# raulmur/ORB_SLAM

Measured on AMD Instinct MI355X. Metric: frames/s ORB extract+match @640x480, 1000 kp, higher is better.
Workload: dtype u8; 1 GPU; vga: 640x480 grayscale stream, 8 levels, nFeatures 1000, S-blocks frames, extract + Hamming top-2 match vs previous frame (BASELINE.json configs[1] + the frame-to-frame match of the metric); resident_frames_per_gpu=2048, lanes=4, parity_checked_frames=0, parity_mismatches=0, library_build_id=255c35022344858e, lane_placement=2

## Files before the change

orb_slam_amd/csrc/k_describe_od.hip:

```cpp
#include <algorithm>
#include <type_traits>

#include "orbx_device.h"

namespace orbx {

constexpr int OD_KPW = 4;
constexpr int OD_PITCH = 48, OD_ROWS = 43;
constexpr int OD_WIN_BYTES = OD_PITCH * OD_ROWS;
constexpr int OD_CHUNKS = OD_ROWS * 3;
constexpr int OD_WAVES = DESC_WAVES;
constexpr int OD_TAIL = 512;

typedef int v4i __attribute__((ext_vector_type(4)));
typedef float f2v __attribute__((ext_vector_type(2)));
__device__ __forceinline__ int float_bits(float v) { return __builtin_bit_cast(int, v); }
typedef const void __attribute__((address_space(1))) * gptr_t;
typedef void __attribute__((address_space(3))) * lptr_t;

constexpr int od_tap(int t) { return t >= 0 && t <= 6 ? (int)((0x12223137312212ull >> (8 * t)) & 255ull) : 0; }
constexpr uint32_t od_taps4(int t0) { return (uint32_t)od_tap(t0) | (uint32_t)od_tap(t0 + 1) << 8 | (uint32_t)od_tap(t0 + 2) << 16 | (uint32_t)od_tap(t0 + 3) << 24; }
struct OdTables {
    uint32_t mask[256];
    float pat[256][4];
    uint32_t trow[3][64][4];
    uint32_t tcol[4][64][4];
};
constexpr uint32_t c_pattern_host[256] = {
#include "orb_pattern_packed.inc"
};
constexpr OdTables make_od_tables() {
    OdTables T{};
    for (int t = 0; t < 256; t++) {
        const int r = t >> 3, c = t & 7;
        const int v = r - HALF_PATCH, av = v < 0 ? -v : v;
        const int um = r < 31 ? (int)((UMAX_NIBBLES >> (4 * (av & 15))) & 15ull) : -1;
        uint32_t mask = 0;
        for (int kk = 0; kk < 4; kk++) {
            const int u = 4 * c + kk - HALF_PATCH;
            if ((u < 0 ? -u : u) <= um) mask |= 0xFFu << (8 * kk);
        }
        T.mask[t] = mask;
        const uint32_t pk = c_pattern_host[t];
        for (int e = 0; e < 4; e++) T.pat[t][e] = (float)(int)(int8_t)(uint8_t)(pk >> (8 * e));
    }
    for (int c = 0; c < 3; c++)
        for (int l = 0; l < 64; l++)
            for (int v = 0; v < 4; v++) {
                const int n = l & 15, g = l >> 4;
                if (c < 2) T.trow[c][l][v] = od_taps4(16 * g + 4 * v - (16 * c + n) - 1);
                else T.trow[c][l][v] = g == 2 && n < 8 ? od_taps4(4 * v - n - 1) : g == 3 && n >= 8 ? od_taps4(4 * v - (n - 8) - 1) : 0u;
            }
    for (int c = 0; c < 4; c++)
        for (int l = 0; l < 64; l++)
            for (int v = 0; v < 4; v++) {
                const int n = l & 15, g = l >> 4;
                uint32_t word = 0;
                for (int h = 0; h < 2; h++) {
                    const int row = 4 * g + 2 * (v >> 1) + h;
                    const int t = c == 0 ? row - n : c == 1 ? 16 + row - n : c == 2 ? (n < 5 ? row - n : -1) : (n >= 8 && n < 13 ? row - (n - 8) : -1);
                    word |= f16_bits_scaled(blur_tap(t), (v & 1) ? 8 : 16) << (16 * h);
                }
                T.tcol[c][l][v] = word;
            }
    return T;
}
static __device__ __constant__ OdTables c_od = make_od_tables();

typedef _Float16 h8v __attribute__((ext_vector_type(8)));
typedef _Float16 h2v __attribute__((ext_vector_type(2)));
typedef float f4v __attribute__((ext_vector_type(4)));
constexpr bool OD_CVT_RNE = true;
constexpr int OD_GEN = 0, OD_EVEN = 1, OD_UP = 2;

struct OdWin { int xs, yq; uint32_t tw; bool gen; };
__device__ __forceinline__ void od_blur_windows(uint8_t* win0, int lane, int nlive, OdWin w0, OdWin w1, OdWin w2, OdWin w3, int Lw, int Lh, int Lwvec, const v4i (&Trow)[3], const v4i (&Tcol)[2], const v4i* tprow) {
    const int n16 = lane & 15, g4 = lane >> 4;
    const unsigned a_off = (unsigned)(n16 * OD_PITCH + 16 * g4);
    const unsigned a_offp = g4 == 3 ? (unsigned)(OD_WIN_BYTES + n16 * OD_PITCH + 32) : a_off;
    const unsigned o_own = (unsigned)((n16 + 3) * OD_PITCH + 4 + 4 * g4);
    const unsigned o_prow = (unsigned)((n16 >= 8 ? OD_WIN_BYTES : 0) + ((n16 & 7) + 35) * OD_PITCH + 4 + 4 * g4);
    const unsigned o_pcol = (unsigned)((g4 >= 2 ? OD_WIN_BYTES : 0) + (n16 + 3) * OD_PITCH + 36 + 4 * (g4 & 1));
    const unsigned o_corner = (unsigned)((n16 < 8 ? 2 : 0) * OD_WIN_BYTES + (g4 >= 2 ? OD_WIN_BYTES : 0) + ((n16 & 7) + 35) * OD_PITCH + 36 + 4 * (g4 & 1));
    const v4i cmid = {blurf_mid_start(), blurf_mid_start(), blurf_mid_start(), blurf_mid_start()};
    const h2v unbias = {(_Float16)-blurf_lo_bias(), (_Float16)-blurf_lo_bias()};
    auto row_pass = [&](const v4i (&A)[3], const v4i& T, v4i (&M)[3]) {
        v4i z[3];
#pragma unroll
        for (int t = 0; t < 3; t++) z[t] = __builtin_amdgcn_mfma_i32_16x16x64_i8(A[t], T, cmid, 0, 0, 0);
#pragma unroll
        for (int t = 0; t < 3; t++)
#pragma unroll
            for (int h = 0; h < 2; h++) {
                const uint32_t z0 = (uint32_t)z[t][2 * h], z1 = (uint32_t)z[t][2 * h + 1];
                M[t][2 * h] = (int)__builtin_amdgcn_perm(z1, z0, 0x06040200u);
                M[t][2 * h + 1] = __builtin_bit_cast(int, __builtin_bit_cast(h2v, __builtin_amdgcn_perm(z1, z0, 0x06050201u)) + unbias);
            }
    };
    auto epilogue = [&](auto MODE, const v4i& Ma, const v4i& Mb, const v4i& Ta, const v4i& Tb, uint8_t* dst, int xs_l, int yq_l, int cb, int ro) {
        constexpr bool gen = decltype(MODE)::value == OD_GEN, twu = decltype(MODE)::value == OD_EVEN;
        constexpr float st = (gen || twu) ? blurf_start() : blurf_start() + 0.5f;
        f4v acc = {st, st, st, st};
        acc = __builtin_amdgcn_mfma_f32_16x16x32_f16(__builtin_bit_cast(h8v, Ma), __builtin_bit_cast(h8v, Ta), acc, 0, 0, 0);
        acc = __builtin_amdgcn_mfma_f32_16x16x32_f16(__builtin_bit_cast(h8v, Mb), __builtin_bit_cast(h8v, Tb), acc, 0, 0, 0);
        float v[4] = {acc[0], acc[1], acc[2], acc[3]};
        uint32_t keep = 0;
        if (gen) {
            const int X0 = xs_l + 4 + cb;
            const bool te = X0 < Lwvec;
            uint32_t keepc = 0;
#pragma unroll
            for (int bb = 0; bb < 4; bb++) keepc |= ((unsigned)(X0 + bb) < (unsigned)Lw ? 0u : 0xFFu) << (8 * bb);
            keep = (unsigned)(yq_l - 18 + ro) < (unsigned)Lh ? keepc : 0xFFFFFFFFu;
#pragma unroll
            for (int i = 0; i < 4; i++) v[i] = te ? __builtin_rintf(v[i]) : __builtin_floorf(v[i] + 0.5f);
        } else if (!twu) {
#pragma unroll
            for (int i = 0; i < 4; i++) v[i] = __builtin_floorf(v[i]);
        } else if (!OD_CVT_RNE) {
#pragma unroll
            for (int i = 0; i < 4; i++) v[i] = __builtin_rintf(v[i]);
        }
        uint32_t o = 0;
#pragma unroll
        for (int i = 0; i < 4; i++) o = __builtin_amdgcn_cvt_pk_u8_f32(v[i], (uint32_t)i, o);
        uint32_t* d = reinterpret_cast<uint32_t*>(dst);
        if (gen) o = (o & ~keep) | (*d & keep);
        *d = o;
    };
    v4i mc[2] = {{0, 0, 0, 0}, {0, 0, 0, 0}};
    auto blur_pair = [&](auto GEN, int p, int xs0, int yq0, int xs1, int yq1) {
        uint8_t* W = win0 + 2 * p * OD_WIN_BYTES;
        v4i A0[3], A1[3];
        {
            const unsigned r0 = (unsigned)(uintptr_t)(lptr_t)(W + a_offp), r1 = (unsigned)(uintptr_t)(lptr_t)(W + OD_WIN_BYTES + a_off);
            asm volatile("ds_read_b128 %0, %6\n\tds_read_b128 %1, %6 offset:768\n\tds_read_b128 %2, %6 offset:1536\n\t"
                         "ds_read_b128 %3, %7\n\tds_read_b128 %4, %7 offset:768\n\tds_read_b128 %5, %7 offset:1536\n\ts_waitcnt lgkmcnt(0)"
                         : "=&v"(A0[0]), "=&v"(A0[1]), "=&v"(A0[2]), "=&v"(A1[0]), "=&v"(A1[1]), "=&v"(A1[2]) : "v"(r0), "v"(r1) : "memory");
        }
#pragma unroll
        for (int t = 0; t < 3; t++)
#pragma unroll
            for (int e = 0; e < 4; e++) { A0[t][e] = (int)((uint32_t)A0[t][e] ^ 0x80808080u); A1[t][e] = (int)((uint32_t)A1[t][e] ^ 0x80808080u); }
        const int xs_r = n16 >= 8 ? xs1 : xs0, yq_r = n16 >= 8 ? yq1 : yq0;
        const int xs_c = g4 >= 2 ? xs1 : xs0, yq_c = g4 >= 2 ? yq1 : yq0;
        {
            v4i MP[3];
            row_pass(A0, Trow[2], MP);
#pragma unroll
            for (int rt = 0; rt < 2; rt++)
                epilogue(GEN, MP[rt], MP[rt + 1], Tcol[0], Tcol[1], W + o_pcol + 16 * rt * OD_PITCH, xs_c, yq_c, 32 + 4 * (g4 & 1), 16 * rt + n16);
            if (p == 0) { mc[0] = MP[2]; mc[1] = MP[2]; }
            else mc[1] = MP[2];
        }
#pragma unroll
        for (int ct = 0; ct < 2; ct++) {
            v4i M0[3], M1[3];
            row_pass(A0, Trow[ct], M0);
#pragma unroll
            for (int rt = 0; rt < 2; rt++)
                epilogue(GEN, M0[rt], M0[rt + 1], Tcol[0], Tcol[1], W + o_own + (16 * rt * OD_PITCH + 16 * ct), xs0, yq0, 16 * ct + 4 * g4, 16 * rt + n16);
            row_pass(A1, Trow[ct], M1);
#pragma unroll
            for (int rt = 0; rt < 2; rt++)
                epilogue(GEN, M1[rt], M1[rt + 1], Tcol[0], Tcol[1], W + OD_WIN_BYTES + o_own + (16 * rt * OD_PITCH + 16 * ct), xs1, yq1, 16 * ct + 4 * g4, 16 * rt + n16);
            epilogue(GEN, M0[2], M1[2], tprow[0], tprow[64], W + o_prow + 16 * ct, xs_r, yq_r, 16 * ct + 4 * g4, 32 + (n16 & 7));
        }
    };
#pragma unroll 1
    for (int p = 0; p < 2; p++) {
        if (p > 0 && nlive <= 2) continue;
        const int xs0 = p ? w2.xs : w0.xs, yq0 = p ? w2.yq : w0.yq, xs1 = p ? w3.xs : w1.xs, yq1 = p ? w3.yq : w1.yq;
        const uint32_t tw0 = p ? w2.tw : w0.tw, tw1 = p ? w3.tw : w1.tw;
        if ((p ? w2.gen || w3.gen : w0.gen || w1.gen) || tw0 != tw1) blur_pair(std::integral_constant<int, OD_GEN>{}, p, xs0, yq0, xs1, yq1);
        else if (tw0) blur_pair(std::integral_constant<int, OD_EVEN>{}, p, xs0, yq0, xs1, yq1);
        else blur_pair(std::integral_constant<int, OD_UP>{}, p, xs0, yq0, xs1, yq1);
    }
    {
        const bool gen = w0.gen || w1.gen || w2.gen || w3.gen || w0.tw != w1.tw || w0.tw != w2.tw || w0.tw != w3.tw;
        const int wsc = (n16 < 8 ? 2 : 0) + (g4 >= 2 ? 1 : 0);
        const int xs_k = wsc == 0 ? w0.xs : wsc == 1 ? w1.xs : wsc == 2 ? w2.xs : w3.xs;
        const int yq_k = wsc == 0 ? w0.yq : wsc == 1 ? w1.yq : wsc == 2 ? w2.yq : w3.yq;
        if (gen) epilogue(std::integral_constant<int, OD_GEN>{}, mc[1], mc[0], tprow[0], tprow[64], win0 + o_corner, xs_k, yq_k, 32 + 4 * (g4 & 1), 32 + (n16 & 7));
        else if (w0.tw) epilogue(std::integral_constant<int, OD_EVEN>{}, mc[1], mc[0], tprow[0], tprow[64], win0 + o_corner, xs_k, yq_k, 32 + 4 * (g4 & 1), 32 + (n16 & 7));
        else epilogue(std::integral_constant<int, OD_UP>{}, mc[1], mc[0], tprow[0], tprow[64], win0 + o_corner, xs_k, yq_k, 32 + 4 * (g4 & 1), 32 + (n16 & 7));
    }
}

template <bool FMA, bool GATHER>
__device__ __forceinline__ void k_describe_od_body(const Batch& b) {
    __shared__ __attribute__((aligned(16))) float s_pat[256 * 4];
    __shared__ __attribute__((aligned(16))) uint32_t s_mask[256];
    __shared__ __attribute__((aligned(16))) uint8_t s_win[OD_WAVES * OD_KPW * OD_WIN_BYTES + OD_TAIL];
    __shared__ __attribute__((aligned(16))) v4i s_tprow[2 * 64];
    const DevGeom& g = b.g;
    int frame, wgi;
    if (!frame_item(b, blockIdx.x, (g.nquads + OD_WAVES - 1) / OD_WAVES, frame, wgi)) return;
    const int tid = threadIdx.x, lane = tid & 63;
    const int grp = lane >> 4, li = lane & 15;
    const float4 pat_first = *reinterpret_cast<const float4*>(c_od.pat[tid & 255]);
    const uint32_t mask_first = c_od.mask[tid & 255];
    const uint2 tprow_first = reinterpret_cast<const uint2*>(c_od.tcol[2])[tid & 255];
    const int32_t* counts = b.level_count + frame * MAX_LEVELS;
    const int quad = wgi * OD_WAVES + wave_id();
    const bool live = quad < g.nquads;
    const int level = __builtin_amdgcn_readfirstlane(find_level(g.quad_bases, live ? quad : 0));
    const LevelGeom& LG = g.lv[level];
    struct { int w, h, stride, plane_off, sel_base, quad_base, wvec; float scale, kp_size; } L = {
        __builtin_amdgcn_readfirstlane(LG.w), __builtin_amdgcn_readfirstlane(LG.h), __builtin_amdgcn_readfirstlane(LG.stride),
        __builtin_amdgcn_readfirstlane(LG.plane_off), __builtin_amdgcn_readfirstlane(LG.sel_base), __builtin_amdgcn_readfirstlane(LG.quad_base),
        __builtin_amdgcn_readfirstlane(LG.blur_wvec),
        __builtin_bit_cast(float, __builtin_amdgcn_readfirstlane(__builtin_bit_cast(int, LG.scale))),
        __builtin_bit_cast(float, __builtin_amdgcn_readfirstlane(__builtin_bit_cast(int, LG.kp_size)))};
    const int k0 = (quad - L.quad_base) * OD_KPW;
    Cand kp;
    typedef int v8i_s __attribute__((ext_vector_type(8)));
    v8i_s s_cnt0, s_cnt1;
    int st0;
    {
        const int sel_cap = __builtin_amdgcn_readfirstlane(LG.sel_cap);
        const int ks = __builtin_amdgcn_readfirstlane(max(min(k0, sel_cap - OD_KPW), 0));
        const Cand* kp4 = b.sel + ((long long)frame * g.frame_sel + L.sel_base + ks);
        const int32_t* stp = b.status + frame;
        static_assert(MAX_LEVELS >= 16, "the per-level counts are fetched as two s_load_dwordx8");
        v8i_s kq;
        int sst;
        asm volatile("s_load_dwordx8 %0, %4, 0x0\n\ts_load_dwordx8 %1, %5, 0x0\n\ts_load_dwordx8 %2, %5, 0x20\n\ts_load_dword %3, %6, 0x0\n\ts_waitcnt lgkmcnt(0)"
                     : "=&s"(kq), "=&s"(s_cnt0), "=&s"(s_cnt1), "=&s"(sst) : "s"(kp4), "s"(counts), "s"(stp) : "memory");
        st0 = sst;
        const int e = min(max(k0 + grp, 0), sel_cap - 1) - ks;
        kp.pos = (uint32_t)(e == 0 ? kq[0] : e == 1 ? kq[2] : e == 2 ? kq[4] : kq[6]);
        kp.resp = __builtin_bit_cast(float, e == 0 ? kq[1] : e == 1 ? kq[3] : e == 2 ? kq[5] : kq[7]);
    }
    static_assert(OD_WAVES * 64 == 256, "one table entry per thread");
    reinterpret_cast<float4*>(s_pat)[tid] = pat_first;
    s_mask[tid] = mask_first;
    reinterpret_cast<uint2*>(s_tprow)[tid] = tprow_first;
    int out_base = 0, total = 0, cnt = 0;
    for (int l = 0; l < g.nlevels; l++) {
        int c = 0;
#pragma unroll
        for (int i = 0; i < 8; i++) { if (l == i) c = s_cnt0[i]; if (l == 8 + i) c = s_cnt1[i]; }
        if (l < level) out_base += c;
        if (l == level) cnt = c;
        total += c;
    }
    const bool work = live && k0 < cnt && total <= b.cap && __builtin_amdgcn_readfirstlane(st0) == ORBX_OK;
    const bool valid = work && k0 + grp < cnt;
    const int k = valid ? k0 + grp : (work ? k0 : 0);
    if (!valid) {
        kp.pos = (uint32_t)__builtin_amdgcn_readlane((int)kp.pos, 0);
        kp.resp = __builtin_bit_cast(float, __builtin_amdgcn_readlane(__builtin_bit_cast(int, kp.resp), 0));
    }
    if (quad == 0 && lane == 0) {
        int st = st0, tot = total;
        if (tot > b.cap) { st = ORBX_ERR_CAPACITY; tot = 0; }
        b.out_n[frame] = st == ORBX_OK ? tot : 0;
        if (b.out_status) b.out_status[frame] = st;
    }
    if (!work) return;
    const int x = kp.pos & 0xFFFF, y = kp.pos >> 16;
    const uint8_t* plain;
    unsigned pstride;
    int wlim;
    if (level == 0) {
        if constexpr (GATHER) {
            long long s0;
            plain = level0_src(b, frame, s0);
            pstride = (unsigned)s0;
        } else { pstride = (unsigned)b.img_row_stride; plain = b.img + (long long)frame * b.img_frame_stride; }
        wlim = (int)min((long long)pstride, (long long)((L.w + 15) & ~15));
    } else { pstride = (unsigned)L.stride; plain = b.pyr + (long long)frame * g.frame_plane_bytes + L.plane_off; wlim = L.stride; }
    uint8_t* const win0 = s_win + wave_id() * OD_KPW * OD_WIN_BYTES;

    int erow[3], ecol[3];
    unsigned eoff[3];
#pragma unroll
    for (int n = 0; n < 3; n++) {
        const int e = 64 * n + lane;
        erow[n] = (e * 171) >> 9;
        ecol[n] = 16 * (e - 3 * erow[n]);
        eoff[n] = __umul24((unsigned)erow[n], pstride) + (unsigned)ecol[n];
    }
    uint32_t fixmask = 0;
#pragma unroll
    for (int q = 0; q < OD_KPW; q++) {
        if (q > 0 && k0 + q >= cnt) continue;
        const unsigned posq = (unsigned)__builtin_amdgcn_readlane((int)kp.pos, 16 * q);
        const int xq = posq & 0xFFFF, yq = posq >> 16;
        const int xs = (xq - 22) & ~3;
        if (xs < 0 || xs + 48 > wlim || xq + 21 >= L.w) fixmask |= 1u << q;
        if (xq < 18 || xq + 18 >= L.w || yq < 18 || yq + 21 >= L.h) fixmask |= 16u << q;
        if (xs >= 0 && xs + 48 <= wlim && yq >= 21 && yq + 21 < L.h) {
            const uint8_t* srcq = plain + (__umul24((unsigned)(yq - 21), pstride) + (unsigned)xs);
#pragma unroll
            for (int n = 0; n < 3; n++)
                if (n < 2 || lane < OD_CHUNKS - 128)
                    __builtin_amdgcn_global_load_lds((gptr_t)(srcq + eoff[n]), (lptr_t)(win0 + q * OD_WIN_BYTES + 1024 * n), 16, 0, 0);
            continue;
        }
#pragma unroll
        for (int n = 0; n < 3; n++) {
            if (n == 2 && lane >= OD_CHUNKS - 128) continue;
            int Y = yq - 21 + erow[n];
            Y = Y < 0 ? -Y : Y;
            Y = Y >= L.h ? 2 * L.h - 2 - Y : Y;
            Y = min(max(Y, 0), L.h - 1);
            const int X = min(max(xs + ecol[n], 0), wlim - 16);
            __builtin_amdgcn_global_load_lds((gptr_t)(plain + (__umul24((unsigned)Y, pstride) + (unsigned)X)), (lptr_t)(win0 + q * OD_WIN_BYTES + 1024 * n), 16, 0, 0);
        }
    }
    fixmask = (uint32_t)__builtin_amdgcn_readfirstlane((int)fixmask);
    asm volatile("s_waitcnt lgkmcnt(0)\n\ts_barrier" ::: "memory");

    v4i Trow[3], Tcol[2];
#pragma unroll
    for (int c = 0; c < 3; c++) Trow[c] = *reinterpret_cast<const v4i*>(c_od.trow[c][lane]);
#pragma unroll
    for (int c = 0; c < 2; c++) Tcol[c] = *reinterpret_cast<const v4i*>(c_od.tcol[c][lane]);
    asm volatile("s_waitcnt vmcnt(0)" ::: "memory");
    wave_lds_fence();

    if (fixmask & 15u) {
#pragma unroll 1
        for (int q = 0; q < OD_KPW; q++) {
            if (!((fixmask >> q) & 1u)) continue;
            const unsigned posq = (unsigned)__builtin_amdgcn_readlane((int)kp.pos, 16 * q);
            const int xq = posq & 0xFFFF;
            const int xs = (xq - 22) & ~3;
            uint8_t* W = win0 + q * OD_WIN_BYTES;
#pragma unroll 1
            for (int j = 0; j < 3; j += 2) {
                const int X0 = xs + 16 * j, Xc = min(max(X0, 0), wlim - 16);
                if (X0 >= 0 && X0 + 16 <= wlim && X0 + 15 < L.w) continue;
                uint32_t nv[3];
#pragma unroll
                for (int it = 0; it < 3; it++) {
                    const int item = 64 * it + lane;
                    const int r = item >> 2, d = item & 3;
                    uint32_t v = 0;
                    if (item < 4 * OD_ROWS) {
#pragma unroll
                        for (int bb = 0; bb < 4; bb++) {
                            const int X = X0 + 4 * d + bb;
                            int Xr = X < 0 ? -X : (X >= L.w ? 2 * L.w - 2 - X : X);
                            Xr = min(max(Xr, 0), L.w - 1);
                            const int src = (Xr >= Xc && Xr < Xc + 16) ? 16 * j + (Xr - Xc) : min(max(Xr - xs, 0), OD_PITCH - 1);
                            v |= (uint32_t)W[r * OD_PITCH + src] << (8 * bb);
                        }
                    }
                    nv[it] = v;
                }
                wave_lds_fence();
#pragma unroll
                for (int it = 0; it < 3; it++) {
                    const int item = 64 * it + lane;
                    if (item < 4 * OD_ROWS) *reinterpret_cast<uint32_t*>(W + (item >> 2) * OD_PITCH + 16 * j + 4 * (item & 3)) = nv[it];
                }
                wave_lds_fence();
            }
        }
    }

    const int xs_own = (x - 22) & ~3, cx = x - xs_own;
    const uint8_t* Wown = win0 + grp * OD_WIN_BYTES;
    int m10, m01;
    {
        const int rsub = li >> 1, hf = li & 1;
        const int boff = cx - HALF_PATCH + 16 * hf;
        const int sh = boff & 3;
        const uint32_t* rowp = reinterpret_cast<const uint32_t*>(Wown + (6 + rsub) * OD_PITCH + (boff & ~3));
        uint32_t uw[4];
#pragma unroll
        for (int d = 0; d < 4; d++) uw[d] = (uint32_t)(16 * hf + 4 * d) * 0x01010101u + 0x03020100u;
        uint32_t a_su = 0, a_si = 0, a_r = 0;
#pragma unroll
        for (int n = 0; n < 4; n++) {
            const uint32_t* p = rowp + (8 * n) * (OD_PITCH / 4);
            uint32_t dw[5];
#pragma unroll
            for (int d = 0; d < 5; d++) dw[d] = p[d];
            const uint4 mk = *reinterpret_cast<const uint4*>(s_mask + (8 * (8 * n + rsub) + 4 * hf));
            const uint32_t mm[4] = {mk.x, mk.y, mk.z, mk.w};
            uint32_t srow = 0;
#pragma unroll
            for (int d = 0; d < 4; d++) {
                const uint32_t Im = __builtin_amdgcn_alignbyte(dw[d + 1], dw[d], (uint32_t)sh) & mm[d];
                srow = __builtin_amdgcn_udot4(Im, 0x01010101u, srow, false);
                a_su = __builtin_amdgcn_udot4(Im, uw[d], a_su, false);
            }
            a_si += srow;
            a_r = __umul24(srow, (uint32_t)(8 * n)) + a_r;
        }
        const int p10 = (int)a_su - HALF_PATCH * (int)a_si;
        const int p01 = (rsub - HALF_PATCH) * (int)a_si + (int)a_r;
        m10 = row16_sum(p10); m01 = row16_sum(p01);
    }
    const float angle = fast_atan2_deg((float)m01, (float)m10);
    wave_lds_fence();

    int xsw[OD_KPW], yqw[OD_KPW];
    uint32_t tww[OD_KPW];
    bool genw[OD_KPW];
#pragma unroll
    for (int q = 0; q < OD_KPW; q++) {
        const unsigned posq = (unsigned)__builtin_amdgcn_readlane((int)kp.pos, 16 * q);
        xsw[q] = ((int)(posq & 0xFFFF) - 22) & ~3;
        yqw[q] = (int)(posq >> 16);
        const bool lo = xsw[q] + 4 < L.wvec, hi = xsw[q] + 40 < L.wvec;
        const bool liveq = q == 0 || k0 + q < cnt;
        tww[q] = liveq ? (lo ? 1u : 0u) : tww[q > 0 ? q - 1 : 0];
        genw[q] = liveq && (((fixmask >> (4 + q)) & 1u) || lo != hi);
    }
    od_blur_windows(win0, lane, min(cnt - k0, OD_KPW), OdWin{xsw[0], yqw[0], tww[0], genw[0]}, OdWin{xsw[1], yqw[1], tww[1], genw[1]},
                    OdWin{xsw[2], yqw[2], tww[2], genw[2]}, OdWin{xsw[3], yqw[3], tww[3], genw[3]}, L.w, L.h, L.wvec, Trow, Tcol, s_tprow + lane);
    wave_lds_fence();

    const float factorPI = (float)(3.14159265358979323846 / 180.f);
    float sn, cs;
    sincosf_orb(angle * factorPI, &sn, &cs);
    const float4* pat = reinterpret_cast<const float4*>(s_pat) + li;
    uint32_t mybits = 0;
    {
        const uint8_t* ctr = Wown + 21 * OD_PITCH + cx;
        const f2v SC = {sn, cs};
        auto rotate = [&](f2v pt) -> f2v {
            f2v m1, r;
            asm("v_pk_mul_f32 %0, %1, %2 op_sel:[1,1] op_sel_hi:[1,0]" : "=v"(m1) : "v"(pt), "v"(SC));
            if (FMA) asm("v_pk_fma_f32 %0, %1, %2, %3 op_sel:[0,0,0] op_sel_hi:[0,1,1] neg_hi:[0,0,1]" : "=v"(r) : "v"(pt), "v"(SC), "v"(m1));
            else {
                f2v m0;
                asm("v_pk_mul_f32 %0, %1, %2 op_sel:[0,0] op_sel_hi:[0,1]" : "=v"(m0) : "v"(pt), "v"(SC));
                asm("v_pk_add_f32 %0, %1, %2 neg_hi:[0,1]" : "=v"(r) : "v"(m0), "v"(m1));
            }
            return r;
        };
        f2v MAGIC = {12582912.0f, 12582912.0f};
        asm("" : "+v"(MAGIC));
        const uint32_t ctr_a = (uint32_t)(uintptr_t)(lptr_t)ctr - (uint32_t)(OD_PITCH * 0x400000 + 0x4B400000);
        typedef const uint8_t __attribute__((address_space(3))) * lbyte_t;
#pragma unroll
        for (int j = 15; j >= 0; j--) {
            const float4 P = pat[16 * j];
            f2v r0 = rotate((f2v){P.x, P.y}), r1 = rotate((f2v){P.z, P.w});
            r0 = r0 + MAGIC;
            r1 = r1 + MAGIC;
            const float r0y = r0.x, r0x = r0.y, r1y = r1.x, r1x = r1.y;
            const uint32_t o0 = (uint32_t)(__mul24(float_bits(r0y), OD_PITCH) + float_bits(r0x));
            const uint32_t o1 = (uint32_t)(__mul24(float_bits(r1y), OD_PITCH) + float_bits(r1x));
            const uint32_t v0 = *(lbyte_t)(uintptr_t)(ctr_a + o0), v1 = *(lbyte_t)(uintptr_t)(ctr_a + o1);
            asm("v_cmp_lt_u32_e32 vcc, %1, %2\n\tv_addc_co_u32_e32 %0, vcc, %0, %0, vcc" : "+v"(mybits) : "v"(v0), "v"(v1) : "vcc");
        }
    }
    uint32_t half = mybits;
    auto stage = [&](auto S) {
        constexpr int s = decltype(S)::value;
        constexpr uint32_t M0 = s == 8 ? 0x00FFu : s == 4 ? 0x0F0Fu : s == 2 ? 0x3333u : 0x5555u;
        const bool hi = (li & s) != 0;
        const uint32_t yv = (uint32_t)__builtin_amdgcn_ds_swizzle((int)half, (s << 10) | 0x1F);
        const uint32_t ysh = hi ? (yv >> s) : (yv << s);
        const uint32_t mk = hi ? (~M0 & 0xFFFFu) : M0;
        half = (half & mk) | (ysh & ~mk & 0xFFFFu);
    };
    stage(std::integral_constant<int, 8>{}); stage(std::integral_constant<int, 4>{});
    stage(std::integral_constant<int, 2>{}); stage(std::integral_constant<int, 1>{});
    if (!valid) return;
    const int out_idx = out_base + k;
    reinterpret_cast<uint16_t*>(b.out_desc + ((long long)frame * b.cap + out_idx) * 32)[li] = (uint16_t)half;
    if (li == 0) {
        orbx_keypoint o;
        o.x = (float)x; o.y = (float)y;
        if (level != 0) { o.x = o.x * L.scale; o.y = o.y * L.scale; }
        o.size = L.kp_size;
        o.angle = angle;
        o.response = kp.resp;
        o.octave = level;
        o.class_id = -1;
        b.out_kps[(long long)frame * b.cap + out_idx] = o;
    }
}
template <bool FMA>
__global__ __launch_bounds__(OD_WAVES * 64) __attribute__((amdgpu_waves_per_eu(4))) void k_describe_od(Batch b) { k_describe_od_body<FMA, false>(b); }
template <bool FMA>
__global__ __launch_bounds__(OD_WAVES * 64) __attribute__((amdgpu_waves_per_eu(4))) void k_describe_od_gather(Batch b) { k_describe_od_body<FMA, true>(b); }

bool describe_od_supported(const Batch& b, const HostGeom& hg) {
    const DevGeom& g = hg.g;
    for (int l = 0; l < g.nlevels; l++)
        if (g.lv[l].w < 64 || g.lv[l].h < 44) return false;
    const long long wlim0 = std::min<long long>(level0_min_stride(b), (g.lv[0].w + 15) & ~15);
    return wlim0 >= 64 && wlim0 >= g.lv[0].w;
}

int launch_describe_od(const Batch& b, const HostGeom& hg, hipStream_t stream) {
    const DevGeom& g = hg.g;
    const dim3 grid(frame_item_blocks(b, (g.nquads + OD_WAVES - 1) / OD_WAVES)), block(OD_WAVES * 64);
    if (g.fp_contract) hipLaunchKernelGGL(b.img_tab ? k_describe_od_gather<true> : k_describe_od<true>, grid, block, 0, stream, b);
    else hipLaunchKernelGGL(b.img_tab ? k_describe_od_gather<false> : k_describe_od<false>, grid, block, 0, stream, b);
    return hipGetLastError() == hipSuccess ? ORBX_OK : ORBX_ERR_DEVICE;
}

__global__ __launch_bounds__(64) void k_eval_blur_window(const uint32_t* win, uint8_t* out, int n, int ties_even, int general) {
    __shared__ __attribute__((aligned(16))) uint32_t s_w[(OD_KPW * OD_WIN_BYTES + OD_TAIL) / 4];
    const int lane = threadIdx.x, q0 = blockIdx.x * OD_KPW, nlive = min(n - q0, OD_KPW);
    for (int i = lane; i < (OD_KPW * OD_WIN_BYTES + OD_TAIL) / 4; i += 64)
        s_w[i] = i < nlive * (OD_WIN_BYTES / 4) ? win[(size_t)q0 * (OD_WIN_BYTES / 4) + i] : 0u;
    __shared__ __attribute__((aligned(16))) v4i s_tprow[2 * 64];
    v4i Trow[3], Tcol[2];
#pragma unroll
    for (int c = 0; c < 3; c++) Trow[c] = *reinterpret_cast<const v4i*>(c_od.trow[c][lane]);
#pragma unroll
    for (int c = 0; c < 2; c++) { Tcol[c] = *reinterpret_cast<const v4i*>(c_od.tcol[c][lane]); s_tprow[64 * c + lane] = *reinterpret_cast<const v4i*>(c_od.tcol[2 + c][lane]); }
    wave_lds_fence();
    const int big = 1 << 20;
    const OdWin w = {0, 18, ties_even ? 1u : 0u, general != 0};
    uint8_t* W = reinterpret_cast<uint8_t*>(s_w);
    od_blur_windows(W, lane, nlive, w, w, w, w, big, big, ties_even ? big : 0, Trow, Tcol, s_tprow + lane);
    wave_lds_fence();
    for (int i = lane; i < nlive * (37 * 40); i += 64) {
        const int q = i / (37 * 40), r = (i - q * (37 * 40)) / 40, c = i % 40;
        out[(size_t)q0 * (37 * 40) + i] = W[q * OD_WIN_BYTES + (r + 3) * OD_PITCH + c + 4];
    }
}
int launch_eval_blur_window(const uint8_t* win, uint8_t* out, int n, int ties_even, int general) {
    static_assert(OD_WIN_BYTES % 4 == 0 && OD_TAIL % 4 == 0, "the windows are copied by dwords");
    hipLaunchKernelGGL(k_eval_blur_window, dim3((n + OD_KPW - 1) / OD_KPW), dim3(64), 0, 0, reinterpret_cast<const uint32_t*>(win), out, n, ties_even, general);
    return hipGetLastError() == hipSuccess ? ORBX_OK : ORBX_ERR_DEVICE;
}

}
```

orb_slam_amd/csrc/orb_math.h:

```cpp
#pragma once
#include <math.h>
#include <stdint.h>

#if defined(__HIPCC__)
#define ORBX_HD __host__ __device__ inline
#else
#define ORBX_HD inline
#endif

namespace orbx {

ORBX_HD int cv_round_f(float v) { return (int)rintf(v); }

ORBX_HD int imin(int a, int b) { return a < b ? a : b; }
ORBX_HD int imax(int a, int b) { return a > b ? a : b; }
ORBX_HD int imin3(int a, int b, int c) { return imin(imin(a, b), c); }
ORBX_HD int imax3(int a, int b, int c) { return imax(imax(a, b), c); }

ORBX_HD int reflect101(int p, int len) {
    if ((unsigned)p < (unsigned)len) return p;
    if (len == 1) return 0;
    do {
        p = p < 0 ? -p : 2 * len - 2 - p;
    } while ((unsigned)p >= (unsigned)len);
    return p;
}

ORBX_HD float fast_atan2_deg(float y, float x) {
    const float k = (float)(180 / 3.14159265358979323846);
    const float p1 = 0.9997878412794807f * k, p3 = -0.3258083974640975f * k;
    const float p5 = 0.1555786518463281f * k, p7 = -0.04432655554792128f * k;
    const float eps = 2.2204460492503131e-16f;
    float ax = fabsf(x), ay = fabsf(y);
    float a, c, c2;
    if (ax >= ay) {
        c = ay / (ax + eps);
        c2 = c * c;
        a = (((p7 * c2 + p5) * c2 + p3) * c2 + p1) * c;
    } else {
        c = ax / (ay + eps);
        c2 = c * c;
        a = 90.f - (((p7 * c2 + p5) * c2 + p3) * c2 + p1) * c;
    }
    if (x < 0) a = 180.f - a;
    if (y < 0) a = 360.f - a;
    return a;
}

ORBX_HD void sincosf_orb(float y, float* sinp, float* cosp) {
    const double hpi_inv = 0x1.45F306DC9C883p+23;
    const double hpi = 0x1.921FB54442D18p0;
    const double c0 = 0x1p0, c1 = -0x1.ffffffd0c621cp-2, c2 = 0x1.55553e1068f19p-5;
    const double c3 = -0x1.6c087e89a359dp-10, c4 = 0x1.99343027bf8c3p-16;
    const double s1 = -0x1.555545995a603p-3, s2 = 0x1.1107605230bc4p-7, s3 = -0x1.994eb3774cf24p-13;
    double x = (double)y;
    int n = 0;
    const float ay = fabsf(y);
    if (!(ay < 0x1.921fb6p-1f)) {
        double r = x * hpi_inv;
        n = ((int32_t)r + 0x800000) >> 24;
        x = x - (double)n * hpi;
    }
    const double x2 = x * x;
    double ps, pc;
    {
        double x3 = x * x2;
        double t1 = s2 + x2 * s3;
        double x7 = x3 * x2;
        double s = x + x3 * s1;
        ps = s + x7 * t1;
    }
    {
        double x4 = x2 * x2;
        double t2 = c3 + x2 * c4;
        double t1 = c0 + x2 * c1;
        double x6 = x4 * x2;
        double c = t1 + x4 * c2;
        pc = c + x6 * t2;
    }
    double sv = (n & 1) ? pc : ps;
    double cv = (n & 1) ? ps : pc;
    if (n & 2) sv = -sv;
    if ((n + 1) & 2) cv = -cv;
    if (n == 0 && ay < 0x1p-12f) sv = (double)y;
    *sinp = (float)sv;
    *cosp = (float)cv;
}

ORBX_HD int fast9_score(const int d[16], int tmin) {
    int lo3[16], hi3[16];
#pragma unroll
    for (int k = 0; k < 16; k++) {
        lo3[k] = imin3(d[k], d[(k + 1) & 15], d[(k + 2) & 15]);
        hi3[k] = imax3(d[k], d[(k + 1) & 15], d[(k + 2) & 15]);
    }
    int dark = -1000, bright = 1000;
#pragma unroll
    for (int k = 0; k < 16; k++) {
        int lo9 = imin3(lo3[k], lo3[(k + 3) & 15], lo3[(k + 6) & 15]);
        int hi9 = imax3(hi3[k], hi3[(k + 3) & 15], hi3[(k + 6) & 15]);
        dark = imax(dark, lo9);
        bright = imin(bright, hi9);
    }
    int s = imax(dark, -bright) - 1;
    return s >= tmin ? s : 0;
}

ORBX_HD int avg_u8(int a, int b, int c) { return (a + b + (c & 1)) >> 1; }
ORBX_HD int compass_t(int t) { return t < 0 ? 0 : t > 254 ? 254 : t; }
ORBX_HD int compass_r(int t) { return compass_t(t) & 1; }
ORBX_HD int compass_kb(int t) { return 128 - (compass_t(t) + compass_r(t)) / 2; }
ORBX_HD int compass_kd(int t) { return 255 - (254 + compass_r(t) - compass_t(t)) / 2; }
ORBX_HD uint32_t avg4_u8(uint32_t a, uint32_t b, uint32_t c) {
    uint32_t o = 0;
    for (int j = 0; j < 4; j++) o |= (uint32_t)avg_u8((int)((a >> (8 * j)) & 255u), (int)((b >> (8 * j)) & 255u), (int)((c >> (8 * j)) & 1u)) << (8 * j);
    return o;
}
ORBX_HD uint32_t compass4_flags(uint32_t C, uint32_t E, uint32_t W, uint32_t N, uint32_t S, int t) {
    const uint32_t R = (uint32_t)compass_r(t) * 0x01010101u, KB = (uint32_t)compass_kb(t) * 0x01010101u, KD = (uint32_t)compass_kd(t) * 0x01010101u;
    const uint32_t nc = ~C;
    const uint32_t hN = avg4_u8(N, nc, R), hS = avg4_u8(S, nc, R), hE = avg4_u8(E, nc, R), hW = avg4_u8(W, nc, R);
    const uint32_t br = (avg4_u8(hN, KB, 0) | avg4_u8(hS, KB, 0)) & (avg4_u8(hE, KB, 0) | avg4_u8(hW, KB, 0));
    const uint32_t dk = (avg4_u8(hN, KD, 0) & avg4_u8(hS, KD, 0)) | (avg4_u8(hE, KD, 0) & avg4_u8(hW, KD, 0));
    return (br | ~dk) & 0x80808080u;
}

ORBX_HD int resize_px(int s00, int s01, int s10, int s11, int a0, int a1, int b0, int b1) {
    int d0 = s00 * a0 + s01 * a1;
    int d1 = s10 * a0 + s11 * a1;
    return (((b0 * (d0 >> 4)) >> 16) + ((b1 * (d1 >> 4)) >> 16) + 2) >> 2;
}

#define ORBX_G0 18
#define ORBX_G1 34
#define ORBX_G2 49
#define ORBX_G3 55
ORBX_HD int blur_taps7(int a, int b, int c, int d, int e, int f, int g) {
    return ORBX_G0 * (a + g) + ORBX_G1 * (b + f) + ORBX_G2 * (c + e) + ORBX_G3 * d;
}
ORBX_HD int blur_round(int sum, int ties_even) {
    int q = (sum + 0x7FFF + (ties_even ? ((sum >> 16) & 1) : 1)) >> 16;
    return q > 255 ? 255 : q;
}

ORBX_HD constexpr int blur_tap(int t) { return t == 0 || t == 6 ? ORBX_G0 : t == 1 || t == 5 ? ORBX_G1 : t == 2 || t == 4 ? ORBX_G2 : t == 3 ? ORBX_G3 : 0; }
ORBX_HD constexpr int blur_tap_sum() { return blur_tap(0) + blur_tap(1) + blur_tap(2) + blur_tap(3) + blur_tap(4) + blur_tap(5) + blur_tap(6); }
ORBX_HD constexpr int blurf_lo_bias() { return 1024; }
ORBX_HD constexpr int blurf_hi(int mid) { return mid >> 8; }
ORBX_HD constexpr int blurf_lo(int mid) { return blurf_lo_bias() + (mid & 255); }
ORBX_HD constexpr float blurf_tap_hi(int t) { return (float)blur_tap(t) / 256.f; }
ORBX_HD constexpr float blurf_tap_lo(int t) { return (float)blur_tap(t) / 65536.f; }
ORBX_HD constexpr float blurf_start() { return -(float)(blurf_lo_bias() * blur_tap_sum()) / 65536.f; }
ORBX_HD constexpr int blurf_mid_start() { return 128 * blur_tap_sum() + (0x64 << 16); }
ORBX_HD constexpr uint32_t f16_bits_scaled(int v, int shift) {
    if (v <= 0) return 0u;
    int p = 0;
    while ((v >> p) > 1) p++;
    return (uint32_t)(p - shift + 15) << 10 | (((uint32_t)v << (10 - p)) & 0x3FFu);
}
ORBX_HD float blurf_column(const int mid[7]) {
    float acc = blurf_start();
    for (int t = 0; t < 7; t++) acc = acc + (float)blurf_hi(mid[t]) * blurf_tap_hi(t);
    for (int t = 0; t < 7; t++) acc = acc + (float)blurf_lo(mid[t]) * blurf_tap_lo(t);
    return acc;
}
ORBX_HD int blurf_round(float v, int ties_even) {
    const float r = ties_even ? rintf(v) : floorf(v + 0.5f);
    return r > 255.f ? 255 : r < 0.f ? 0 : (int)r;
}

ORBX_HD int hamming256_words(const uint32_t* a, const uint32_t* b) {
    int dist = 0;
    for (int i = 0; i < 8; i++) {
        dist += __builtin_popcount(a[i] ^ b[i]);
    }
    return dist;
}

}
```

Measured before the change: 485,100 frames/s.

## Interleave blur MFMAs with epilogues and hide orientation math inside blur

Splits the row pass into an MFMA stage and a separate split stage, then software-pipelines them so the next row MFMA is issued while the previous tile's epilogue runs. The atan2 and sincos for keypoint orientation move inside the first blur pair so their ALU work can overlap MFMA latency. Table loads for Trow/Tcol are hoisted earlier to overlap with global loads, and fast_atan2 becomes branchless. This raises register pressure and adds template instantiations.

```diff
diff --git a/orb_slam_amd/csrc/k_describe_od.hip b/orb_slam_amd/csrc/k_describe_od.hip
--- a/orb_slam_amd/csrc/k_describe_od.hip
+++ b/orb_slam_amd/csrc/k_describe_od.hip
@@ -74,7 +74,9 @@
 constexpr int OD_GEN = 0, OD_EVEN = 1, OD_UP = 2;
 
 struct OdWin { int xs, yq; uint32_t tw; bool gen; };
-__device__ __forceinline__ void od_blur_windows(uint8_t* win0, int lane, int nlive, OdWin w0, OdWin w1, OdWin w2, OdWin w3, int Lw, int Lh, int Lwvec, const v4i (&Trow)[3], const v4i (&Tcol)[2], const v4i* tprow) {
+struct OdAngle { int m01, m10; float angle, sn, cs; };
+template <class ANG>
+__device__ __forceinline__ void od_blur_windows(ANG, OdAngle& ang, uint8_t* win0, int lane, int nlive, OdWin w0, OdWin w1, OdWin w2, OdWin w3, int Lw, int Lh, int Lwvec, const v4i (&Trow)[3], const v4i (&Tcol)[2], const v4i* tprow) {
     const int n16 = lane & 15, g4 = lane >> 4;
     const unsigned a_off = (unsigned)(n16 * OD_PITCH + 16 * g4);
     const unsigned a_offp = g4 == 3 ? (unsigned)(OD_WIN_BYTES + n16 * OD_PITCH + 32) : a_off;
@@ -84,15 +86,16 @@
     const unsigned o_corner = (unsigned)((n16 < 8 ? 2 : 0) * OD_WIN_BYTES + (g4 >= 2 ? OD_WIN_BYTES : 0) + ((n16 & 7) + 35) * OD_PITCH + 36 + 4 * (g4 & 1));
     const v4i cmid = {blurf_mid_start(), blurf_mid_start(), blurf_mid_start(), blurf_mid_start()};
     const h2v unbias = {(_Float16)-blurf_lo_bias(), (_Float16)-blurf_lo_bias()};
-    auto row_pass = [&](const v4i (&A)[3], const v4i& T, v4i (&M)[3]) {
-        v4i z[3];
-#pragma unroll
-        for (int t = 0; t < 3; t++) z[t] = __builtin_amdgcn_mfma_i32_16x16x64_i8(A[t], T, cmid, 0, 0, 0);
+    auto row_mm = [&](const v4i (&A)[3], const v4i& T, v4i (&M)[3]) {
+#pragma unroll
+        for (int t = 0; t < 3; t++) M[t] = __builtin_amdgcn_mfma_i32_16x16x64_i8(A[t], T, cmid, 0, 0, 0);
+    };
+    auto row_split = [&](v4i (&M)[3]) {
 #pragma unroll
         for (int t = 0; t < 3; t++)
 #pragma unroll
             for (int h = 0; h < 2; h++) {
-                const uint32_t z0 = (uint32_t)z[t][2 * h], z1 = (uint32_t)z[t][2 * h + 1];
+                const uint32_t z0 = (uint32_t)M[t][2 * h], z1 = (uint32_t)M[t][2 * h + 1];
                 M[t][2 * h] = (int)__builtin_amdgcn_perm(z1, z0, 0x06040200u);
                 M[t][2 * h + 1] = __builtin_bit_cast(int, __builtin_bit_cast(h2v, __builtin_amdgcn_perm(z1, z0, 0x06050201u)) + unbias);
             }
@@ -129,7 +132,8 @@
         *d = o;
     };
     v4i mc[2] = {{0, 0, 0, 0}, {0, 0, 0, 0}};
-    auto blur_pair = [&](auto GEN, int p, int xs0, int yq0, int xs1, int yq1) {
+    auto blur_pair = [&](auto GEN, auto P, int xs0, int yq0, int xs1, int yq1) {
+        constexpr int p = decltype(P)::value;
         uint8_t* W = win0 + 2 * p * OD_WIN_BYTES;
         v4i A0[3], A1[3];
         {
@@ -144,46 +148,53 @@
             for (int e = 0; e < 4; e++) { A0[t][e] = (int)((uint32_t)A0[t][e] ^ 0x80808080u); A1[t][e] = (int)((uint32_t)A1[t][e] ^ 0x80808080u); }
         const int xs_r = n16 >= 8 ? xs1 : xs0, yq_r = n16 >= 8 ? yq1 : yq0;
         const int xs_c = g4 >= 2 ? xs1 : xs0, yq_c = g4 >= 2 ? yq1 : yq0;
-        {
-            v4i MP[3];
-            row_pass(A0, Trow[2], MP);
-#pragma unroll
-            for (int rt = 0; rt < 2; rt++)
-                epilogue(GEN, MP[rt], MP[rt + 1], Tcol[0], Tcol[1], W + o_pcol + 16 * rt * OD_PITCH, xs_c, yq_c, 32 + 4 * (g4 & 1), 16 * rt + n16);
-            if (p == 0) { mc[0] = MP[2]; mc[1] = MP[2]; }
-            else mc[1] = MP[2];
-        }
+        v4i MP[3], M0[3], M1[3];
+        const int cbo = 4 * g4, cbp = 32 + 4 * (g4 & 1);
+        row_mm(A0, Trow[2], MP);
+        if constexpr (p == 0 && ANG::value) ang.angle = fast_atan2_deg((float)ang.m01, (float)ang.m10);
+        row_split(MP);
+        epilogue(GEN, MP[0], MP[1], Tcol[0], Tcol[1], W + o_pcol, xs_c, yq_c, cbp, n16);
+        row_mm(A0, Trow[0], M0);
+        epilogue(GEN, MP[1], MP[2], Tcol[0], Tcol[1], W + o_pcol + 16 * OD_PITCH, xs_c, yq_c, cbp, 16 + n16);
+        if (p == 0) { mc[0] = MP[2]; mc[1] = MP[2]; }
+        else mc[1] = MP[2];
 #pragma unroll
         for (int ct = 0; ct < 2; ct++) {
-            v4i M0[3], M1[3];
-            row_pass(A0, Trow[ct], M0);
-#pragma unroll
-            for (int rt = 0; rt < 2; rt++)
-                epilogue(GEN, M0[rt], M0[rt + 1], Tcol[0], Tcol[1], W + o_own + (16 * rt * OD_PITCH + 16 * ct), xs0, yq0, 16 * ct + 4 * g4, 16 * rt + n16);
-            row_pass(A1, Trow[ct], M1);
-#pragma unroll
-            for (int rt = 0; rt < 2; rt++)
-                epilogue(GEN, M1[rt], M1[rt + 1], Tcol[0], Tcol[1], W + OD_WIN_BYTES + o_own + (16 * rt * OD_PITCH + 16 * ct), xs1, yq1, 16 * ct + 4 * g4, 16 * rt + n16);
-            epilogue(GEN, M0[2], M1[2], tprow[0], tprow[64], W + o_prow + 16 * ct, xs_r, yq_r, 16 * ct + 4 * g4, 32 + (n16 & 7));
+            uint8_t* const d0 = W + o_own + 16 * ct, * const d1 = d0 + OD_WIN_BYTES;
+            row_split(M0);
+            epilogue(GEN, M0[0], M0[1], Tcol[0], Tcol[1], d0, xs0, yq0, 16 * ct + cbo, n16);
+            row_mm(A1, Trow[ct], M1);
+            epilogue(GEN, M0[1], M0[2], Tcol[0], Tcol[1], d0 + 16 * OD_PITCH, xs0, yq0, 16 * ct + cbo, 16 + n16);
+            row_split(M1);
+            epilogue(GEN, M1[0], M1[1], Tcol[0], Tcol[1], d1, xs1, yq1, 16 * ct + cbo, n16);
+            epilogue(GEN, M1[1], M1[2], Tcol[0], Tcol[1], d1 + 16 * OD_PITCH, xs1, yq1, 16 * ct + cbo, 16 + n16);
+            const v4i m02 = M0[2];
+            const v4i tp0 = tprow[0], tp1 = tprow[64];
+            if (ct == 0) row_mm(A0, Trow[1], M0);
+            epilogue(GEN, m02, M1[2], tp0, tp1, W + o_prow + 16 * ct, xs_r, yq_r, 16 * ct + cbo, 32 + (n16 & 7));
+            if constexpr (p == 0 && ANG::value)
+                if (ct == 0) sincosf_orb(ang.angle * (float)(3.14159265358979323846 / 180.f), &ang.sn, &ang.cs);
         }
     };
-#pragma unroll 1
-    for (int p = 0; p < 2; p++) {
-        if (p > 0 && nlive <= 2) continue;
-        const int xs0 = p ? w2.xs : w0.xs, yq0 = p ? w2.yq : w0.yq, xs1 = p ? w3.xs : w1.xs, yq1 = p ? w3.yq : w1.yq;
-        const uint32_t tw0 = p ? w2.tw : w0.tw, tw1 = p ? w3.tw : w1.tw;
-        if ((p ? w2.gen || w3.gen : w0.gen || w1.gen) || tw0 != tw1) blur_pair(std::integral_constant<int, OD_GEN>{}, p, xs0, yq0, xs1, yq1);
-        else if (tw0) blur_pair(std::integral_constant<int, OD_EVEN>{}, p, xs0, yq0, xs1, yq1);
-        else blur_pair(std::integral_constant<int, OD_UP>{}, p, xs0, yq0, xs1, yq1);
-    }
+    auto blur_pair_of = [&](auto P, const OdWin& wa, const OdWin& wb) {
+        if (wa.gen || wb.gen || wa.tw != wb.tw) blur_pair(std::integral_constant<int, OD_GEN>{}, P, wa.xs, wa.yq, wb.xs, wb.yq);
+        else if (wa.tw) blur_pair(std::integral_constant<int, OD_EVEN>{}, P, wa.xs, wa.yq, wb.xs, wb.yq);
+        else blur_pair(std::integral_constant<int, OD_UP>{}, P, wa.xs, wa.yq, wb.xs, wb.yq);
+    };
+    blur_pair_of(std::integral_constant<int, 0>{}, w0, w1);
+    if (nlive > 2) blur_pair_of(std::integral_constant<int, 1>{}, w2, w3);
     {
         const bool gen = w0.gen || w1.gen || w2.gen || w3.gen || w0.tw != w1.tw || w0.tw != w2.tw || w0.tw != w3.tw;
         const int wsc = (n16 < 8 ? 2 : 0) + (g4 >= 2 ? 1 : 0);
         const int xs_k = wsc == 0 ? w0.xs : wsc == 1 ? w1.xs : wsc == 2 ? w2.xs : w3.xs;
         const int yq_k = wsc == 0 ? w0.yq : wsc == 1 ? w1.yq : wsc == 2 ? w2.yq : w3.yq;
-        if (gen) epilogue(std::integral_constant<int, OD_GEN>{}, mc[1], mc[0], tprow[0], tprow[64], win0 + o_corner, xs_k, yq_k, 32 + 4 * (g4 & 1), 32 + (n16 & 7));
-        else if (w0.tw) epilogue(std::integral_constant<int, OD_EVEN>{}, mc[1], mc[0], tprow[0], tprow[64], win0 + o_corner, xs_k, yq_k, 32 + 4 * (g4 & 1), 32 + (n16 & 7));
-        else epilogue(std::integral_constant<int, OD_UP>{}, mc[1], mc[0], tprow[0], tprow[64], win0 + o_corner, xs_k, yq_k, 32 + 4 * (g4 & 1), 32 + (n16 & 7));
+        auto corner = [&](auto MODE) {
+            const v4i tp0 = tprow[0], tp1 = tprow[64];
+            epilogue(MODE, mc[1], mc[0], tp0, tp1, win0 + o_corner, xs_k, yq_k, 32 + 4 * (g4 & 1), 32 + (n16 & 7));
+        };
+        if (gen) corner(std::integral_constant<int, OD_GEN>{});
+        else if (w0.tw) corner(std::integral_constant<int, OD_EVEN>{});
+        else corner(std::integral_constant<int, OD_UP>{});
     }
 }
 
@@ -259,6 +270,11 @@
         if (b.out_status) b.out_status[frame] = st;
     }
     if (!work) return;
+    v4i Trow[3], Tcol[2];
+#pragma unroll
+    for (int c = 0; c < 3; c++) Trow[c] = *reinterpret_cast<const v4i*>(c_od.trow[c][lane]);
+#pragma unroll
+    for (int c = 0; c < 2; c++) Tcol[c] = *reinterpret_cast<const v4i*>(c_od.tcol[c][lane]);
     const int x = kp.pos & 0xFFFF, y = kp.pos >> 16;
     const uint8_t* plain;
     unsigned pstride;
@@ -313,11 +329,6 @@
     fixmask = (uint32_t)__builtin_amdgcn_readfirstlane((int)fixmask);
     asm volatile("s_waitcnt lgkmcnt(0)\n\ts_barrier" ::: "memory");
 
-    v4i Trow[3], Tcol[2];
-#pragma unroll
-    for (int c = 0; c < 3; c++) Trow[c] = *reinterpret_cast<const v4i*>(c_od.trow[c][lane]);
-#pragma unroll
-    for (int c = 0; c < 2; c++) Tcol[c] = *reinterpret_cast<const v4i*>(c_od.tcol[c][lane]);
     asm volatile("s_waitcnt vmcnt(0)" ::: "memory");
     wave_lds_fence();
 
@@ -396,7 +407,7 @@
         const int p01 = (rsub - HALF_PATCH) * (int)a_si + (int)a_r;
         m10 = row16_sum(p10); m01 = row16_sum(p01);
     }
-    const float angle = fast_atan2_deg((float)m01, (float)m10);
+    OdAngle ang = {m01, m10, 0.f, 0.f, 0.f};
     wave_lds_fence();
 
     int xsw[OD_KPW], yqw[OD_KPW];
@@ -412,13 +423,11 @@
         tww[q] = liveq ? (lo ? 1u : 0u) : tww[q > 0 ? q - 1 : 0];
         genw[q] = liveq && (((fixmask >> (4 + q)) & 1u) || lo != hi);
     }
-    od_blur_windows(win0, lane, min(cnt - k0, OD_KPW), OdWin{xsw[0], yqw[0], tww[0], genw[0]}, OdWin{xsw[1], yqw[1], tww[1], genw[1]},
+    od_blur_windows(std::true_type{}, ang, win0, lane, min(cnt - k0, OD_KPW), OdWin{xsw[0], yqw[0], tww[0], genw[0]}, OdWin{xsw[1], yqw[1], tww[1], genw[1]},
                     OdWin{xsw[2], yqw[2], tww[2], genw[2]}, OdWin{xsw[3], yqw[3], tww[3], genw[3]}, L.w, L.h, L.wvec, Trow, Tcol, s_tprow + lane);
     wave_lds_fence();
 
-    const float factorPI = (float)(3.14159265358979323846 / 180.f);
-    float sn, cs;
-    sincosf_orb(angle * factorPI, &sn, &cs);
+    const float angle = ang.angle, sn = ang.sn, cs = ang.cs;
     const float4* pat = reinterpret_cast<const float4*>(s_pat) + li;
     uint32_t mybits = 0;
     {
@@ -515,7 +524,8 @@
     const int big = 1 << 20;
     const OdWin w = {0, 18, ties_even ? 1u : 0u, general != 0};
     uint8_t* W = reinterpret_cast<uint8_t*>(s_w);
-    od_blur_windows(W, lane, nlive, w, w, w, w, big, big, ties_even ? big : 0, Trow, Tcol, s_tprow + lane);
+    OdAngle noang = {0, 0, 0.f, 0.f, 0.f};
+    od_blur_windows(std::false_type{}, noang, W, lane, nlive, w, w, w, w, big, big, ties_even ? big : 0, Trow, Tcol, s_tprow + lane);
     wave_lds_fence();
     for (int i = lane; i < nlive * (37 * 40); i += 64) {
         const int q = i / (37 * 40), r = (i - q * (37 * 40)) / 40, c = i % 40;
diff --git a/orb_slam_amd/csrc/orb_math.h b/orb_slam_amd/csrc/orb_math.h
--- a/orb_slam_amd/csrc/orb_math.h
+++ b/orb_slam_amd/csrc/orb_math.h
@@ -32,16 +32,11 @@
     const float p5 = 0.1555786518463281f * k, p7 = -0.04432655554792128f * k;
     const float eps = 2.2204460492503131e-16f;
     float ax = fabsf(x), ay = fabsf(y);
-    float a, c, c2;
-    if (ax >= ay) {
-        c = ay / (ax + eps);
-        c2 = c * c;
-        a = (((p7 * c2 + p5) * c2 + p3) * c2 + p1) * c;
-    } else {
-        c = ax / (ay + eps);
-        c2 = c * c;
-        a = 90.f - (((p7 * c2 + p5) * c2 + p3) * c2 + p1) * c;
-    }
+    const bool xg = ax >= ay;
+    const float c = (xg ? ay : ax) / ((xg ? ax : ay) + eps);
+    const float c2 = c * c;
+    float a = (((p7 * c2 + p5) * c2 + p3) * c2 + p1) * c;
+    if (!xg) a = 90.f - a;
     if (x < 0) a = 180.f - a;
     if (y < 0) a = 360.f - a;
     return a;
```

New measurement: 485,900 frames/s, median of 3. Within noise of the previous version (+0.2%).
